# flo-audio/flo

Hardware: AMD Instinct MI355X
Metric: Msamples/s encoded (44.1k stereo, q=high) (higher is better)
Workload: dtype f32

## Files before the change

### flo_amd/csrc/context.cpp

```cpp
#include <cstdio>
#include <cstdlib>
#include <cstring>

#include "ctx_internal.hpp"

thread_local std::string g_create_err;

int fail(flo_ctx *c, int code, const std::string &msg) {
    if (c) c->err = msg;
    return code;
}

extern "C" const char *flo_last_create_error(void) { return g_create_err.c_str(); }
extern "C" const char *flo_last_error(const flo_ctx *ctx) { return ctx ? ctx->err.c_str() : "null context"; }
extern "C" void flo_free(void *p) { free(p); }

extern "C" int flo_ctx_create(int device, flo_ctx **out) {
    if (!out) return FLO_ERR_ARG;
    *out = nullptr;
    int n = 0;
    hipError_t e = hipGetDeviceCount(&n);
    if (e != hipSuccess || n == 0) {
        g_create_err = std::string("no HIP device available: ") + (e != hipSuccess ? hipGetErrorString(e) : "count = 0") +
                       " (libflo_hip has no CPU fallback)";
        return FLO_ERR_DEVICE;
    }
    if (device < 0 || device >= n) {
        g_create_err = "device index out of range";
        return FLO_ERR_ARG;
    }
    flo_ctx *c = new flo_ctx();
    c->device = device;
    int prev_dev = -1;
    hipGetDevice(&prev_dev);
    auto restore = [&] {
        if (prev_dev >= 0 && prev_dev != device) hipSetDevice(prev_dev);
    };
    if ((e = hipSetDevice(device)) != hipSuccess || (e = hipGetDeviceProperties(&c->prop, device)) != hipSuccess ||
        (e = hipStreamCreateWithFlags(&c->stream, hipStreamNonBlocking)) != hipSuccess) {
        g_create_err = std::string("device init failed: ") + hipGetErrorString(e);
        delete c;
        restore();
        return FLO_ERR_DEVICE;
    }
    if (std::string(c->prop.gcnArchName).find("gfx950") == std::string::npos) {
        g_create_err = std::string("device is ") + c->prop.gcnArchName + ", this library carries gfx950 code only";
        hipStreamDestroy(c->stream);
        delete c;
        restore();
        return FLO_ERR_DEVICE;
    }
    {
        std::string serr;
        c->stager = stager_create(serr);
    }
    if (const char *e2 = getenv("FLO_RESERVE_CUS")) {
        const int v = atoi(e2);
// ... 97 lines not shown
        if (t->host.sample_rate == sr && t->host.quality == q) {
            *out = t;
            return FLO_OK;
        }
    TableSet *t = new TableSet();
    build_lossy_tables(sr, q, t->host);
    const LossyTablesHost &h = t->host;
    struct Part {
        const void *src;
        size_t bytes;
        size_t off;
    };
    std::vector<Part> parts;
    size_t total = 0;
    auto add = [&](const void *p, size_t b) {
        total = (total + 255) & ~(size_t)255;
        parts.push_back({p, b, total});
        total += b;
        return parts.size() - 1;
    };
    size_t i_ext = add(h.pack_ext.data(), h.pack_ext.size() * 4);
    size_t i_pack = add(h.pack.data(), h.pack.size() * 4), i_athdb = add(h.ath_db.data(), h.ath_db.size() * 4),
           i_band = add(h.band.data(), h.band.size()), i_bc = add(h.band_count.data(), h.band_count.size() * 4),
           i_s10 = add(h.s10d.data(), h.s10d.size() * 4), i_lb = add(h.lane_bnd.data(), h.lane_bnd.size() * 4),
           i_ls = add(h.lane_slot0.data(), h.lane_slot0.size() * 4), i_bs = add(h.band_slot0.data(), h.band_slot0.size() * 4),
           i_win = add(h.window.data(), h.window.size() * 4);
    hipError_t e = hipMalloc(&t->blob, total);
    if (e != hipSuccess) {
        delete t;
        return fail(c, FLO_ERR_NOMEM, std::string("hipMalloc tables: ") + hipGetErrorString(e));
    }
    std::vector<uint8_t> stage(total, 0);
    for (auto &p : parts) memcpy(stage.data() + p.off, p.src, p.bytes);
    e = hipMemcpy(t->blob, stage.data(), total, hipMemcpyHostToDevice);
    if (e != hipSuccess) {
        hipFree(t->blob);
        delete t;
        return fail(c, FLO_ERR_DEVICE, std::string("hipMemcpy tables: ") + hipGetErrorString(e));
    }
    auto P = [&](size_t i) { return (const char *)t->blob + parts[i].off; };
    t->dev.pack = (const float4 *)P(i_pack);
    t->dev.pack_g = t->dev.pack;
    t->dev.pack_ext = (const float4 *)P(i_ext);
    t->dev.ath_db = (const float *)P(i_athdb);
    t->dev.band = (const uint8_t *)P(i_band);
    t->dev.band_count = (const float *)P(i_bc);
    t->dev.s10d = (const float *)P(i_s10);
    t->dev.lane_bnd = (const uint32_t *)P(i_lb);
    t->dev.lane_slot0 = (const uint32_t *)P(i_ls);
    t->dev.band_slot0 = (const uint32_t *)P(i_bs);
    t->dev_window = (const float *)P(i_win);
    t->dev.max_band_slots = h.max_band_slots;
    t->dev.dirty = h.dirty;
    t->dev.smr_thr = h.smr_threshold;
    t->dev.q_transparent = h.q_transparent;
    if (h.n_slots > kSlotCap || h.max_band_slots > 64) {
        hipFree(t->blob);
        delete t;
        return fail(c, FLO_ERR_ARG, "band segment table exceeds capacity");
    }
    c->tables.push_back(t);
    *out = t;
    return FLO_OK;
}

int ctx_stager(flo_ctx *c) {
    if (c->stager && c->up_stream) return FLO_OK;
    if (c->stager) {
        HIPCHK(c, hipStreamCreateWithFlags(&c->up_stream, hipStreamNonBlocking));
        HIPCHK(c, hipStreamCreateWithFlags(&c->down_stream, hipStreamNonBlocking));
        return FLO_OK;
    }
    std::string err;
    c->stager = stager_create(err);
    if (!c->stager) return fail(c, FLO_ERR_NOMEM, err);
    HIPCHK(c, hipStreamCreateWithFlags(&c->up_stream, hipStreamNonBlocking));
    HIPCHK(c, hipStreamCreateWithFlags(&c->down_stream, hipStreamNonBlocking));
    return FLO_OK;
}

extern "C" int flo_ctx_reserve_cus(flo_ctx *c, int n) {
    if (!c || n < 0 || n >= c->prop.multiProcessorCount) return FLO_ERR_ARG;
    c->reserve_cus = n;
    return FLO_OK;
}
extern "C" int flo_ctx_upload_path(flo_ctx *c, char *name, size_t cap, double *direct_gbs, double *ring_gbs) {
    if (!c) return FLO_ERR_ARG;
    int rc = ctx_stager(c);
    if (rc != FLO_OK) return rc;
    const char *n = stager_upload_choice(c->stager, direct_gbs, ring_gbs);
    if (name && cap) snprintf(name, cap, "%s", n);
    return FLO_OK;
}
extern "C" int flo_ctx_reserved_cus(flo_ctx *c) { return c ? (c->reserve_cus > 0 ? c->reserve_cus : 0) : -1; }
```

### flo_amd/csrc/encode_plan.hpp

```cpp
#pragma once
#include <cstddef>
#include <cstdint>

namespace flo {

constexpr size_t kFewClips = 64;
constexpr size_t kFusedCompactClips = 16;
constexpr size_t kCoefHandoverBytes = (size_t)256 << 20;
constexpr uint32_t kDirty44k = 0xBDBEu;

enum class LossyForm : uint8_t {
    Chain2q = 5,
    Chain = 1,
    Frames = 2,
};
enum class Chain2qKernel : uint8_t {
    None,
    InCoeffs,
    Debug,
    Dirty44k,
    Generic,
};
enum class ChainKernel : uint8_t {
    None,
    Mono,
    MonoExact,
    Stereo,
    StereoExact,
};
enum class FrameKernel : uint8_t {
    None,
    Mono1, Mono2, Mono2Exact,
    Stereo1, Stereo2, Stereo2Exact,
    Pair1, Pair2,
    Pair2FromCoef,
    Multi1, Multi2, Multi2Exact,
};
enum class CompactKernel : uint8_t {
    None,
    Fused,
    Offsets1024,
    Offsets256,
};

struct LossyPlanInput {
    int which = 0;
    int force_path = 0;
    unsigned ch = 0;
    size_t n_clips = 0;
    uint64_t total_frames = 0;
    bool exact = false, in_coeffs = false;
    bool debug = false;
    uint32_t dirty = 0;
    bool tail_crc = true;
    int chain2q_clips = 0;
};

struct LossyPlan {
    LossyForm form = LossyForm::Chain;
    Chain2qKernel chain2q = Chain2qKernel::None;
    int chain2q_clips = 0;
    ChainKernel chain = ChainKernel::None;
// ... 21 lines not shown
```

### flo_amd/csrc/lossy_device.hpp

```cpp
#pragma once
#include <hip/hip_runtime.h>
#include <stdint.h>

#include "pack_rows.h"

namespace flo {


struct LossyDevTables {
    const float4 *pack;
    const float4 *pack_g;
    const float4 *pack_ext;
    const float *ath_db;
    const uint8_t *band;
    const float *band_count;
    const float *s10d;
    const uint32_t *lane_bnd;
    const uint32_t *lane_slot0;
    const uint32_t *band_slot0;
    int max_band_slots;
    uint32_t dirty;
    float smr_thr;
    int q_transparent;
};

constexpr int kXchStride = 9;
constexpr int kXchFloats = 64 * kXchStride * 2;
#ifdef FLO_COEF_PAD16
constexpr int kCoefFloats = 1280;
#else
constexpr int kCoefFloats = 1152;
#endif
constexpr int kSlotCap = 96;
constexpr int kFrameCap = 4352;

template <int CH>
struct WaveLds {
    union {
        float xch[CH][kXchFloats];
        float coef[CH][kCoefFloats];
        int16_t qbuf[CH][1024];
    } u;
    float2 slots[CH][kSlotCap + 64 + 1];
    float2 bandv[CH][32];
    float band_s[CH][32];
};

__device__ __forceinline__ float4 pack_row(const float4 *p) {
    typedef float v4f __attribute__((ext_vector_type(4)));
    v4f v = *reinterpret_cast<const v4f *>(p);
    asm("" : "+v"(v));
    return make_float4(v.x, v.y, v.z, v.w);
}

__device__ __forceinline__ int lane_id() { return (int)(threadIdx.x & 63); }
__device__ __forceinline__ int lane_id_opaque() {
    int l = (int)(threadIdx.x & 63);
    asm volatile("" : "+v"(l));
    return l;
}

__device__ __forceinline__ void wave_sync() {
    asm volatile("" ::: "memory");
    __builtin_amdgcn_wave_barrier();
    asm volatile("" ::: "memory");
}
__device__ __forceinline__ void lds_barrier() {
    asm volatile("s_waitcnt lgkmcnt(0)\n\ts_barrier" ::: "memory");
}

__device__ __forceinline__ float max_raw(float a, float b) {
    float r;
    asm("v_max_f32 %0, %1, %2" : "=v"(r) : "v"(a), "v"(b));
    return r;
}
__device__ __forceinline__ float max_abs_raw(float a, float b) {
// ... 954 lines not shown
#pragma unroll
    for (int g = 0; g < 4; g++) {
        const float4 al4 = T.pack[(kRowAth + g) * 64 + lane];
        const float4 bo4 = R.bo4[g];
        const float al[4] = {al4.x, al4.y, al4.z, al4.w};
        const uint32_t bo[4] = {__float_as_uint(bo4.x), __float_as_uint(bo4.y), __float_as_uint(bo4.z), __float_as_uint(bo4.w)};
        v4f tb[4];
#pragma unroll
        for (int k = 0; k < 4; k++) tb[k] = *reinterpret_cast<const lds_f4 *>((uintptr_t)(ts0 + 2u * bo[k]));
        int v[2][4];
        float t[2][4];
#pragma unroll
        for (int k = 0; k < 4; k++) {
            const v2f x = c[4 * g + k];
            const v2f xsc = x * (v2f){tb[k].z, tb[k].w};
            uint32_t h0, h1;
            asm("v_bfi_b32 %0, %1, %2, %3" : "=v"(h0) : "s"(sgn_mask), "v"(phalf), "v"(x.x));
            asm("v_bfi_b32 %0, %1, %2, %3" : "=v"(h1) : "s"(sgn_mask), "v"(phalf), "v"(x.y));
            const v2f rs = xsc + (v2f){__uint_as_float(h0), __uint_as_float(h1)};
            v[0][k] = cvt_rz(rs.x);
            v[1][k] = cvt_rz(rs.y);
            t[0][k] = max_raw(tb[k].x, al[k]);
            t[1][k] = max_raw(tb[k].y, al[k]);
        }
#pragma unroll
        for (int ch = 0; ch < 2; ch++)
#pragma unroll
            for (int k2 = 0; k2 < 2; k2++) {
                const float xe = ch ? c[4 * g + 2 * k2].y : c[4 * g + 2 * k2].x;
                const float xo = ch ? c[4 * g + 2 * k2 + 1].y : c[4 * g + 2 * k2 + 1].x;
                uint32_t r;
                asm("v_cmp_gt_f32_e64 vcc, |%1|, %2\n\t"
                    "v_cndmask_b32_e32 %0, 0, %3, vcc\n\t"
                    "v_cmp_gt_f32_e64 vcc, |%4|, %5\n\t"
                    "v_cndmask_b32_sdwa %0, 0, %6, vcc dst_sel:WORD_1 dst_unused:UNUSED_PRESERVE src0_sel:DWORD src1_sel:DWORD"
                    : "=&v"(r)
                    : "v"(xe), "v"(t[ch][2 * k2]), "v"(v[ch][2 * k2]), "v"(xo), "v"(t[ch][2 * k2 + 1]), "v"(v[ch][2 * k2 + 1])
                    : "vcc");
                xs[ch][2 * g + k2] = r;
            }
    }
}

typedef float v4f __attribute__((ext_vector_type(4)));
template <int TSOFF>
__device__ __forceinline__ void quantise_nat(const v4f (&cf)[8], const uint32_t (&ts_a)[16], const float (&athn)[16],
                                             const uint32_t alive, const uint32_t (&blk)[8], uint32_t (&xd)[2][8]) {
    typedef __attribute__((address_space(3))) v4f lds_f4;
    const uint32_t sgn_mask = 0x7FFFFFFFu;
    uint32_t phalf = 0x3EFFFFFFu;
    asm volatile("" : "+v"(phalf));
    auto block = [&](const int k, const v4f t0, const v4f t1, uint32_t &out0, uint32_t &out1) __attribute__((always_inline)) {
        const v2f x0 = {cf[k].x, cf[k].y}, x1 = {cf[k].z, cf[k].w};
        const v2f s0 = x0 * (v2f){t0.z, t0.w}, s1 = x1 * (v2f){t1.z, t1.w};
        uint32_t h00, h01, h10, h11;
        asm("v_bfi_b32 %0, %1, %2, %3" : "=v"(h00) : "s"(sgn_mask), "v"(phalf), "v"(x0.x));
        asm("v_bfi_b32 %0, %1, %2, %3" : "=v"(h01) : "s"(sgn_mask), "v"(phalf), "v"(x0.y));
        asm("v_bfi_b32 %0, %1, %2, %3" : "=v"(h10) : "s"(sgn_mask), "v"(phalf), "v"(x1.x));
        asm("v_bfi_b32 %0, %1, %2, %3" : "=v"(h11) : "s"(sgn_mask), "v"(phalf), "v"(x1.y));
        const v2f r0 = s0 + (v2f){__uint_as_float(h00), __uint_as_float(h01)};
        const v2f r1 = s1 + (v2f){__uint_as_float(h10), __uint_as_float(h11)};
        const int v0[2] = {cvt_rz(r0.x), cvt_rz(r0.y)}, v1[2] = {cvt_rz(r1.x), cvt_rz(r1.y)};
        const float a0 = athn[2 * k], a1 = athn[2 * k + 1];
        const float th0[2] = {max_raw(t0.x, a0), max_raw(t0.y, a0)}, th1[2] = {max_raw(t1.x, a1), max_raw(t1.y, a1)};
        uint32_t r[2];
#pragma unroll
        for (int ch = 0; ch < 2; ch++) {
            const float xe = ch ? x0.y : x0.x, xo = ch ? x1.y : x1.x;
            asm("v_cmp_gt_f32_e64 vcc, |%1|, %2\n\t"
                "v_cndmask_b32_e32 %0, 0, %3, vcc\n\t"
                "v_cmp_gt_f32_e64 vcc, |%4|, %5\n\t"
                "v_cndmask_b32_sdwa %0, 0, %6, vcc dst_sel:WORD_1 dst_unused:UNUSED_PRESERVE src0_sel:DWORD src1_sel:DWORD"
                : "=&v"(r[ch])
                : "v"(xe), "v"(th0[ch]), "v"(v0[ch]), "v"(xo), "v"(th1[ch]), "v"(v1[ch])
                : "vcc");
        }
        out0 = r[0];
        out1 = r[1];
    };
#pragma unroll
    for (int g = 0; g < 4; g++) {
        uint32_t o00 = 0u, o01 = 0u, o10 = 0u, o11 = 0u;
        if (alive & (blk[2 * g] | blk[2 * g + 1])) {
            v4f tb[4];
#pragma unroll
            for (int j = 0; j < 4; j++) tb[j] = *reinterpret_cast<const lds_f4 *>((uintptr_t)(ts_a[4 * g + j] + (uint32_t)TSOFF));
            if (alive & blk[2 * g]) block(2 * g, tb[0], tb[1], o00, o01);
            if (alive & blk[2 * g + 1]) block(2 * g + 1, tb[2], tb[3], o10, o11);
        }
        xd[0][2 * g] = o00, xd[1][2 * g] = o01;
        xd[0][2 * g + 1] = o10, xd[1][2 * g + 1] = o11;
    }
}

__device__ __forceinline__ uint32_t nonzero_mask16(const int (&q)[16]) {
    uint32_t m = 0;
#pragma unroll
    for (int e = 0; e < 16; e++) m |= (q[e] != 0 ? 1u : 0u) << e;
    return m;
}
__device__ __forceinline__ uint32_t nonzero_mask16_packed(const uint32_t (&x)[8], const uint32_t (&hi)[8]) {
    uint32_t m = 0;
#pragma unroll
    for (int k = 0; k < 8; k++) {
        m |= ((x[k] & 0xFFFFu) != 0u ? 1u : 0u) << (2 * k);
        m |= (hi[k] != 0u ? 1u : 0u) << (2 * k + 1);
    }
    return m;
}
__device__ __forceinline__ uint32_t wave_incl_sum(uint32_t x) {
    int v = (int)x;
    v += dpp_i<0x111>(0, v);
    v += dpp_i<0x112>(0, v);
    v += dpp_i<0x114>(0, v);
    v += dpp_i<0x118>(0, v);
    v += dpp_i<0x142, 0xA>(0, v);
    v += dpp_i<0x143, 0xC>(0, v);
    return (uint32_t)v;
}

struct SparsePlan {
    uint32_t M;
    int nn;
    int nz_end;
    uint32_t cross_cnt;
    uint32_t off0;
    uint32_t total;
};

__device__ __forceinline__ void sparse_plan_m(const int lane, const uint32_t m, SparsePlan &P) {
    const uint32_t prev_m = (uint32_t)dpp_i<0x138>(0, (int)m);
    const uint32_t prev_nz = (prev_m >> 15) & 1u;
    uint32_t zs = ~m & ((m << 1) | prev_nz) & 0xFFFFu;
    if (lane == 0 && !(m & 1u)) zs |= 1u;
    const int base = 16 * lane;
    const uint32_t inv = ~m & 0xFFFFu;
    const int first_nz = m ? base + __builtin_ctz(m) : 1024;
    const int first_z = inv ? base + __builtin_ctz(inv) : 1024;
    const int last_z = inv ? base + 31 - __builtin_clz(inv) : -1;
    const unsigned long long has_nz = __ballot(m != 0u), has_z = __ballot(inv != 0u);
    const unsigned long long nz_above = (has_nz >> 1) >> lane, z_above = (has_z >> 1) >> lane;
// ... 405 lines not shown
```

### flo_amd/csrc/lossy_kernels.hip

```cpp
#include <assert.h>
#include <stdlib.h>

#include <mutex>
#include <set>
#include <type_traits>
#include <utility>

#include "crc_device.hpp"
#include "lossy_device.hpp"
#include "lossy_kernels.hpp"
#include "../../include/flo_synth.h"

#ifndef FLO_ABLATE
#define FLO_ABLATE 0
#endif
#ifndef FLO_SKIP
#define FLO_SKIP 0
#endif
#ifndef FLO_ABLATE3
#define FLO_ABLATE3 0
#endif
#define FLO_KEEP(x) asm volatile("" ::"v"(x))
#ifdef FLO_STAMPS
#define STAMP(i)                                                                                  \
// ... 283 lines not shown
        STAMP(4);
#if FLO_ABLATE >= 2
        FLO_KEEP(P[0].total); FLO_KEEP(P[0].off0); FLO_KEEP(P[0].M); FLO_KEEP(sfw[0]);
        for (int e = 0; e < 16; e++) FLO_KEEP(q[0][e]);
        return;
#endif
        uint32_t tot[2];
        if (NW > 1) {
            if (ln == 0) cs.tot[w] = P[0].total;
            pair_sync(cs.cnt, w, ++step);
            STAMP(5);
            tot[0] = cs.tot[0];
            tot[1] = cs.tot[1];
        } else {
            wave_sync();
            tot[0] = P[0].total;
            tot[1] = 0u;
        }
        if (ptid < (int)pend) stage[ptid] = (uint8_t)tailb;
        const uint32_t flen = emit_frame<1>(ln, stage + pend, NW, w, tot, sfw, P, q);
        STAMP(6);
#if FLO_ABLATE >= 1
        FLO_KEEP(flen);
        return;
#endif
        if (NW > 1) pair_sync(cs.cnt, w, ++step); else wave_sync();
        STAMP(7);
        if (ptid == 0) A.frame_size[frame0 + h] = flen;
        const uint32_t have = pend + flen;
        const uint32_t n16 = have >> 4;
        const uint4 *src = reinterpret_cast<const uint4 *>(stage);
        uint4 *dst = reinterpret_cast<uint4 *>(gout + written);
        for (uint32_t i = ptid; i < n16; i += 64 * NW) dst[i] = src[i];
        pend = have & 15u;
        tailb = (ptid < (int)pend) ? stage[(n16 << 4) + ptid] : 0u;
        written += (unsigned long long)n16 << 4;
        STAMP(8);
    };
    for (unsigned h = 0; h < hops; h += 2) {
        frame_body(h, ae, ao, be, bo);
        if (h + 1 < hops) frame_body(h + 1, be, bo, ae, ao);
    }
    if (ptid < (int)pend) gout[written + ptid] = (uint8_t)tailb;
    if (ptid == 0) A.clip_bytes[clip] = written + pend;
#ifdef FLO_STAMPS
    if (A.dbg_stamps && lane == 0)
        for (int i = 0; i < 14; i++) A.dbg_stamps[((unsigned long long)clip * NW + w) * 16 + i] = st_sum[i];
#endif
}

template <int SLEEP = 1>
__device__ __forceinline__ void wait_counter(const uint32_t *p, uint32_t want) {
    const uint32_t a = (uint32_t)(uintptr_t)p;
    uint32_t seen;
    do {
        asm volatile("ds_read_b32 %0, %1\n\ts_waitcnt lgkmcnt(0)" : "=v"(seen) : "v"(a) : "memory");
        if (seen >= want) break;
        __builtin_amdgcn_s_sleep(SLEEP);
    } while (true);
}
__device__ __forceinline__ uint32_t peek_counter(const uint32_t *p) {
    typedef volatile __attribute__((address_space(3))) uint32_t lds_vu32;
    return *reinterpret_cast<lds_vu32 *>((uintptr_t)(uint32_t)(uintptr_t)p);
}
__device__ __forceinline__ void set_counter(uint32_t *p, uint32_t v) {
    const uint32_t a = (uint32_t)(uintptr_t)p;
    asm volatile("ds_write_b32 %0, %1" ::"v"(a), "v"(v) : "memory");
}

#ifndef FLO_C2X_THREADS
#define FLO_C2X_THREADS 768
#endif
#ifdef FLO_MARKS
#define FLO_MARK(x) asm volatile("; MARK " x ::: "memory")
#else
#define FLO_MARK(x)
#endif

struct Clip2qLds {
    union {
        float4 xch4[kXch4];
        float2 coef2[kCoef2];
    } u;
    float4 slot[kSlots];
    float4 ts[2][32];
    __attribute__((aligned(16))) uint8_t stage[kFrameCap + 64 + 256];
    uint16_t sfwh[2][2][32];
    uint32_t alive[2][2];
    uint32_t pad2[4];
    uint32_t packtab[kPackTabDwords];
    uint32_t coef_ready;
    uint32_t ts_ready;
    uint32_t consumed;
    uint32_t clip_seq;
    uint32_t clip_cur;
    uint32_t pad[3];
};
static_assert(sizeof(Clip2qLds) % 16 == 0, "clip LDS block keeps 16-byte alignment");
constexpr int kPackBytesHotT = kPackRowsHotT * 64 * 16;

#ifndef FLO_PSLEEP
#define FLO_PSLEEP 1
#endif
static_assert(sizeof(Clip2qLds::u) >= 8 * 256 * sizeof(uint32_t), "the tail's CRC tables fit the exchange buffer");

__device__ __forceinline__ void tail_publish(const LossyArgs &A, const unsigned clip, const int lane) {
    asm volatile("s_waitcnt vmcnt(0)" ::: "memory");
    if (lane == 0) {
        __builtin_amdgcn_fence(__ATOMIC_RELEASE, "agent");
        asm volatile("s_waitcnt vmcnt(0)" ::: "memory");
        const unsigned slot = __hip_atomic_fetch_add(A.next_clip + 1, 1u, __ATOMIC_RELAXED, __HIP_MEMORY_SCOPE_AGENT);
        if (slot < (unsigned)A.n_clips)
// ... 37 lines not shown
                if (h < (unsigned)A.n_clips) e = __hip_atomic_load(A.done_q + h, __ATOMIC_RELAXED, __HIP_MEMORY_SCOPE_AGENT);
            }
        }
        const unsigned tag = (unsigned)__builtin_amdgcn_readfirstlane((int)(unsigned)(e >> 32));
        clip = (unsigned)__builtin_amdgcn_readfirstlane((int)(unsigned)e);
        if (tag != A.epoch || clip >= (unsigned)A.n_clips) return;
        __builtin_amdgcn_fence(__ATOMIC_ACQUIRE, "agent");
        asm volatile("s_waitcnt vmcnt(0)" ::: "memory");
        total = __hip_atomic_load(A.clip_bytes + clip, __ATOMIC_RELAXED, __HIP_MEMORY_SCOPE_AGENT);
    }
}

template <bool COEFFS, uint32_t DIRTY, bool DBG>
__global__ __launch_bounds__(FLO_C2X_THREADS) void lossy_chain2q_kernel(LossyArgs A, int clips_per_wg) {
    extern __shared__ __attribute__((aligned(16))) uint8_t lds_raw[];
    const int tid = (int)threadIdx.x;
    const int lane = tid & 63;
    {
        float4 *dstp = reinterpret_cast<float4 *>(lds_raw);
        for (int i = tid; i < kPackRowsHotT * 64; i += (int)blockDim.x) dstp[i] = A.T.pack[i];
        for (int i = tid; i < clips_per_wg; i += (int)blockDim.x) {
            Clip2qLds &c0 = *reinterpret_cast<Clip2qLds *>(lds_raw + kPackBytesHotT + (size_t)i * sizeof(Clip2qLds));
            c0.coef_ready = 0;
            c0.ts_ready = 0;
            c0.consumed = 0;
            c0.clip_seq = 0;
        }
        if (A.clear_next && blockIdx.x == 0 && tid == 0)
            A.clear_next[0] = A.clear_next[1] = A.clear_next[2] = 0;
    }
    __syncthreads();
    const int wv = __builtin_amdgcn_readfirstlane(tid >> 6);
    const int cl = wv % clips_per_wg;
    Clip2qLds &cs = *reinterpret_cast<Clip2qLds *>(lds_raw + kPackBytesHotT + (size_t)cl * sizeof(Clip2qLds));
    uint32_t fbase = 0, seq = 0;
    if (wv >= clips_per_wg) {
#ifndef FLO_PRIO_P
#define FLO_PRIO_P 1
#endif
        __builtin_amdgcn_s_setprio(FLO_PRIO_P);
        typedef __attribute__((address_space(3))) v4f lds_v4f;
        float athn[16];
        uint32_t ts_a[16];
        {
            const uint32_t ts0 = (uint32_t)(uintptr_t)cs.ts[0];
#pragma unroll
            for (int q = 0; q < 4; q++) {
                const float4 a4 = A.T.pack[(kRowAthN + q) * 64 + lane];
                const float4 b4 = A.T.pack[(kRowBoN + q) * 64 + lane];
                athn[4 * q + 0] = a4.x, athn[4 * q + 1] = a4.y, athn[4 * q + 2] = a4.z, athn[4 * q + 3] = a4.w;
                ts_a[4 * q + 0] = ts0 + __float_as_uint(b4.x), ts_a[4 * q + 1] = ts0 + __float_as_uint(b4.y);
                ts_a[4 * q + 2] = ts0 + __float_as_uint(b4.z), ts_a[4 * q + 3] = ts0 + __float_as_uint(b4.w);
            }
        }
        const uint32_t *const blk_g = reinterpret_cast<const uint32_t *>(A.T.pack + kRowBlk * 64);
        const uint32_t cf_a = (uint32_t)(uintptr_t)cs.u.coef2 + 16u * (uint32_t)lane + 16u * ((uint32_t)lane >> 3);
        uint8_t *const stage = cs.stage;
        const uint32_t tab_a = (uint32_t)(uintptr_t)cs.packtab;
        v4f cf[8];
        bool have = false;
        unsigned done_clip = ~0u;
        unsigned long long done_bytes = 0;
        for (;;) {
            unsigned got = 0;
            if (lane == 0) got = atomicAdd(A.next_clip, 1u);
            const unsigned clip = (unsigned)__builtin_amdgcn_readfirstlane((int)got);
            if (lane == 0) cs.clip_cur = clip;
            set_counter(&cs.clip_seq, ++seq);
            if (A.crc_ready) {
                if (clip >= (unsigned)A.n_clips) {
                    tail_crc(A, reinterpret_cast<uint32_t *>(&cs.u), lane, done_clip, done_bytes);
                    return;
                }
                if (done_clip != ~0u) tail_publish(A, done_clip, lane);
            }
            if (clip >= (unsigned)A.n_clips) return;
            const unsigned hops = A.clip_hops[clip];
            const unsigned long long frame0 = A.clip_frame0[clip];
            uint8_t *gout = A.out + A.out_off[clip];
            unsigned long long written = 0;
            uint32_t pend = 0, tailb = 0;
#ifdef FLO_STAMPS
            unsigned long long st_sum[16] = {0, 0, 0, 0, 0, 0, 0, 0, 0, 0, 0, 0, 0, 0, 0, 0}, st_last;
            asm volatile("s_memtime %0\n\ts_waitcnt lgkmcnt(0)" : "=s"(st_last)::"memory");
#endif
            for (unsigned h = 0; h < hops; h++) {
                const int ln = lane_id_opaque();
                const uint32_t g = fbase + h;
                auto take_next = [&]() __attribute__((always_inline)) {
                    if (!have && (uint32_t)__builtin_amdgcn_readfirstlane((int)peek_counter(&cs.coef_ready)) >= g + 2) {
#pragma unroll
                        for (int k = 0; k < 8; k++) cf[k] = *reinterpret_cast<const lds_v4f *>((uintptr_t)(cf_a + 1152u * (uint32_t)k));
                        set_counter(&cs.consumed, g + 2);
                        have = true;
                    }
                };
                uint32_t blk[8];
                {
                    const uint32_t *bp = blk_g;
                    asm volatile("" : "+s"(bp));
#pragma unroll
                    for (int q = 0; q < 8; q++) blk[q] = bp[q];
                }
                if (!have) {
                    wait_counter<FLO_PSLEEP>(&cs.coef_ready, g + 1);
#pragma unroll
                    for (int k = 0; k < 8; k++) cf[k] = *reinterpret_cast<const lds_v4f *>((uintptr_t)(cf_a + 1152u * (uint32_t)k));
                    set_counter(&cs.consumed, g + 1);
                }
                STAMP(0);
#ifdef FLO_STAMPS
                const unsigned long long st_frame0 = st_last;
#endif
                wait_counter<FLO_PSLEEP>(&cs.ts_ready, g + 1);
                STAMP(5);
                const uint32_t par = g & 1u;
                const uint32_t sfw_both = cs.sfwh[par][ln >> 5][ln & 31];
                const uint32_t alive = (uint32_t)__builtin_amdgcn_readfirstlane((int)(cs.alive[par][0] | cs.alive[par][1]));
                uint32_t xd[2][8];
#if (FLO_SKIP & 64) == 0
                if (par) quantise_nat<512>(cf, ts_a, athn, alive, blk, xd);
                else quantise_nat<0>(cf, ts_a, athn, alive, blk, xd);
#else
#pragma unroll
                for (int q = 0; q < 8; q++) { xd[0][q] = __float_as_uint(cf[q].x) & alive & 0x00010001u; xd[1][q] = __float_as_uint(cf[q].y) & blk[q] & 0x00010001u; }
#endif
                have = false;
                take_next();
                STAMP(1);
                if (DBG && A.dbg_q) {
#pragma unroll
                    for (int ch = 0; ch < 2; ch++) {
                        uint32_t *dq = reinterpret_cast<uint32_t *>(A.dbg_q + ((frame0 + h) * 2 + ch) * 1024);
#pragma unroll
                        for (int k = 0; k < 8; k++) dq[64 * k + ln] = xd[ch][k];
                    }
                }
                if (ln < (int)pend) stage[ln] = (uint8_t)tailb;
                uint8_t *f = stage + pend;
                const uint32_t f_a = (uint32_t)(uintptr_t)f;
                if ((ln & 31) < 25) {
                    uint8_t *p = f + 12 + 50 * (ln >> 5) + 2 * (ln & 31);
                    lds_st8<0>(p, sfw_both);
                    lds_st8<1>(p, sfw_both >> 8);
                }
                uint32_t tot[2];
                uint32_t pos = 112;
#pragma unroll
                for (int ch = 0; ch < 2; ch++) {
#if (FLO_SKIP & 32) == 0
                    uint32_t t = sparse_item_pack(ln, xd[ch], f_a + pos + 4u, tab_a);
#ifdef FLO_STAMPS
                    if (t == kSparseFallback) st_sum[6] += 1;
#endif
                    if (t == kSparseFallback) t = sparse_block_pack(ln, xd[ch], f_a + pos + 4u, tab_a);
// ... 1020 lines not shown
    hipError_t e = hipGetDevice(&dev);
    if (e != hipSuccess) return (int)e;
    std::lock_guard<std::mutex> g(mu);
    if (done.count({dev, fn})) return 0;
    e = hipFuncSetAttribute(fn, hipFuncAttributeMaxDynamicSharedMemorySize, 160 * 1024);
    if (e != hipSuccess) return (int)e;
    done.insert({dev, fn});
    return 0;
}

int chain_clips_per_wg(int n_clips) {
    int g = (n_clips + 255) / 256;
    const int gmax = (int)((160 * 1024 - kPackBytes) / sizeof(ClipLds));
    if (g > gmax) g = gmax;
    if (g * 2 * 64 > 768) g = 6;
    return g < 1 ? 1 : g;
}

template <int NW, bool EXACT>
static int launch_chain_t(const LossyArgs &A, hipStream_t s) {
    const int g = chain_clips_per_wg(A.n_clips);
    const size_t lds = kPackBytes + (size_t)g * sizeof(ClipLds);
    if (int rc = allow_big_lds(reinterpret_cast<const void *>(&lossy_chain_kernel<NW, EXACT>))) return rc;
    const unsigned wgs = (unsigned)((A.n_clips + g - 1) / g);
    hipLaunchKernelGGL((lossy_chain_kernel<NW, EXACT>), dim3(wgs), dim3(64 * NW * g), lds, s, A, g);
    FLO_LAUNCH_CHECK();
    return 0;
}

int chain2q_clips_per_wg(int n_clips) {
    int g = (n_clips + 255) / 256;
    const int gmax = (int)((160 * 1024 - kPackBytesHotT) / sizeof(Clip2qLds));
    if (g > gmax) g = gmax;
    if (g > FLO_C2X_THREADS / 128) g = FLO_C2X_THREADS / 128;
    return g < 1 ? 1 : g;
}
template <bool COEFFS, uint32_t DIRTY, bool DBG>
static int launch_chain2q_t(const LossyArgs &A, int clips, hipStream_t s) {
    int g = chain2q_clips_per_wg(A.n_clips);
    if (clips >= 1 && clips <= FLO_C2X_THREADS / 128) g = clips;
    const size_t lds = kPackBytesHotT + (size_t)g * sizeof(Clip2qLds);
    if (int rc = allow_big_lds(reinterpret_cast<const void *>(&lossy_chain2q_kernel<COEFFS, DIRTY, DBG>))) return rc;
    unsigned wgs = (unsigned)((A.n_clips + g - 1) / g);
    if (A.n_cus > 0 && wgs > (unsigned)A.n_cus) wgs = (unsigned)A.n_cus;
    hipLaunchKernelGGL((lossy_chain2q_kernel<COEFFS, DIRTY, DBG>), dim3(wgs), dim3(128 * g), lds, s, A, g);
    FLO_LAUNCH_CHECK();
    return 0;
}
int launch_lossy_chain2q(const LossyArgs &A, const LossyPlan &P, hipStream_t s) {
    assert(P.form == LossyForm::Chain2q && A.nch == 2 && !A.exact);
    switch (P.chain2q) {
    case Chain2qKernel::InCoeffs: return launch_chain2q_t<true, 0xFFFFu, true>(A, P.chain2q_clips, s);
    case Chain2qKernel::Debug: return launch_chain2q_t<false, 0xFFFFu, true>(A, P.chain2q_clips, s);
    case Chain2qKernel::Dirty44k: return launch_chain2q_t<false, kDirty44k, false>(A, P.chain2q_clips, s);
    case Chain2qKernel::Generic: return launch_chain2q_t<false, 0xFFFFu, false>(A, P.chain2q_clips, s);
    default: return -1;
    }
}
int launch_lossy_chain(const LossyArgs &A, const LossyPlan &P, hipStream_t s) {
    switch (P.chain) {
    case ChainKernel::Mono: return launch_chain_t<1, false>(A, s);
    case ChainKernel::MonoExact: return launch_chain_t<1, true>(A, s);
    case ChainKernel::Stereo: return launch_chain_t<2, false>(A, s);
    case ChainKernel::StereoExact: return launch_chain_t<2, true>(A, s);
    default: return -1;
    }
}
int launch_lossy_frames_pass(const LossyArgs &A, FrameKernel k, hipStream_t s) {
    dim3 g((unsigned)A.total_frames), b(64);
    const size_t dynb = (size_t)A.slot_bytes + 256 + (size_t)A.nch * 2048;
    switch (k) {
    case FrameKernel::Mono1: hipLaunchKernelGGL((lossy_frame_kernel<1, 1, false>), g, b, 0, s, A); break;
    case FrameKernel::Mono2: hipLaunchKernelGGL((lossy_frame_kernel<1, 2, false>), g, b, 0, s, A); break;
    case FrameKernel::Mono2Exact: hipLaunchKernelGGL((lossy_frame_kernel<1, 2, true>), g, b, 0, s, A); break;
    case FrameKernel::Stereo1: hipLaunchKernelGGL((lossy_frame_kernel<2, 1, false>), g, b, 0, s, A); break;
    case FrameKernel::Stereo2: hipLaunchKernelGGL((lossy_frame_kernel<2, 2, false>), g, b, 0, s, A); break;
    case FrameKernel::Stereo2Exact: hipLaunchKernelGGL((lossy_frame_kernel<2, 2, true>), g, b, 0, s, A); break;
    case FrameKernel::Pair1: hipLaunchKernelGGL((lossy_frame2x_kernel<1>), g, b, 0, s, A); break;
    case FrameKernel::Pair2: hipLaunchKernelGGL((lossy_frame2x_kernel<2>), g, b, 0, s, A); break;
    case FrameKernel::Pair2FromCoef: hipLaunchKernelGGL((lossy_frame2x_kernel<2, true>), g, b, 0, s, A); break;
    case FrameKernel::Multi1: hipLaunchKernelGGL((lossy_frame_n_kernel<1, false>), g, b, dynb, s, A); break;
    case FrameKernel::Multi2: hipLaunchKernelGGL((lossy_frame_n_kernel<2, false>), g, b, dynb, s, A); break;
    case FrameKernel::Multi2Exact: hipLaunchKernelGGL((lossy_frame_n_kernel<2, true>), g, b, dynb, s, A); break;
    default: return -1;
    }
    FLO_LAUNCH_CHECK();
    return 0;
}
int launch_lossy_stream_pass(const LossyArgs &A, int pass, hipStream_t s) {
    dim3 g((unsigned)A.total_frames), b(64);
    const size_t dynb = (size_t)A.slot_bytes + 256 + (size_t)A.nch * 2048;
    constexpr int S1 = 1 | kStreamStep, S2 = 2 | kStreamStep;
    if (A.nch == 1) {
        if (pass == 1) hipLaunchKernelGGL((lossy_frame_kernel<1, S1, false>), g, b, 0, s, A);
        else if (A.exact) hipLaunchKernelGGL((lossy_frame_kernel<1, S2, true>), g, b, 0, s, A);
        else hipLaunchKernelGGL((lossy_frame_kernel<1, S2, false>), g, b, 0, s, A);
    } else if (A.nch == 2 && A.exact) {
        if (pass == 1) hipLaunchKernelGGL((lossy_frame_kernel<2, S1, false>), g, b, 0, s, A);
        else hipLaunchKernelGGL((lossy_frame_kernel<2, S2, true>), g, b, 0, s, A);
    } else if (A.nch == 2) {
        if (pass == 1) hipLaunchKernelGGL((lossy_frame2x_kernel<S1>), g, b, 0, s, A);
        else hipLaunchKernelGGL((lossy_frame2x_kernel<S2>), g, b, 0, s, A);
    } else if (A.nch <= kMaxLossyChannels) {
        if (pass == 1) hipLaunchKernelGGL((lossy_frame_n_kernel<S1, false>), g, b, dynb, s, A);
        else if (A.exact) hipLaunchKernelGGL((lossy_frame_n_kernel<S2, true>), g, b, dynb, s, A);
        else hipLaunchKernelGGL((lossy_frame_n_kernel<S2, false>), g, b, dynb, s, A);
    } else {
// ... 74 lines not shown
```

Before: 658,000.

## Specialise 44k block masks as constants and tighten quantiser and wait-loop codegen

For the 44.1k dirty-band kernel variant, the per-frame block masks become compile-time constants instead of being loaded from global memory. The host checks the table against these constants and falls back to the generic kernel on a mismatch. The quantiser block is rewritten as one interleaved asm sequence that uses separate SGPR masks, to cut vcc serialisation. The counter wait loop moves into scalar-branch asm using readfirstlane, which avoids divergent exec-mask handling. A diagnostic script for counting issue slots is also added.

```diff
diff --git a/diag/issue_slots.py b/diag/issue_slots.py
--- /dev/null
+++ b/diag/issue_slots.py
@@ -0,0 +1,118 @@
+#!/usr/bin/env python3
+import collections
+import re
+import sys
+
+BLOCK = re.compile(r"^(\.LBB\d+_\d+):|^; %bb\.\d+:")
+
+
+def classify(op):
+    if op == "s_nop":
+        return "s_nop"
+    if op.startswith("v_"):
+        return "vector"
+    if op.startswith("ds_"):
+        return "lds"
+    if op.startswith("s_waitcnt"):
+        return "wait"
+    if op.startswith(("global_", "buffer_", "flat_", "scratch_")):
+        return "vmem"
+    if op.startswith(("s_load", "s_buffer_load")):
+        return "smem"
+    if op.startswith("s_"):
+        return "scalar"
+    return None
+
+
+def blocks_of(lines):
+    out = [(None, "", [])]
+    for l in lines:
+        m = BLOCK.match(l)
+        if m:
+            out.append((m.group(1), l.split(";", 1)[1] if ";" in l else "", []))
+            continue
+        s = l.strip()
+        if not s:
+            continue
+        if s.startswith(";"):
+            if not s.startswith(";;#") and not out[-1][2]:
+                out[-1] = (out[-1][0], out[-1][1] + " " + s, out[-1][2])
+            continue
+        if s.startswith((".", "//")) or s.endswith(":"):
+            continue
+        out[-1][2].append(s)
+    return out
+
+
+def loop_blocks(blocks, header):
+    pat = re.compile(r"\b" + re.escape(header.lstrip(".L")) + r"\b")
+    return [b for b in blocks if b[0] == header or pat.search(b[1])]
+
+
+def depth2_header(block):
+    if "This Loop Header: Depth=2" in block[1]:
+        return block[0]
+    m = re.search(r"Header=(BB\d+_\d+) Depth=2", block[1]) or re.search(r"Parent Loop (BB\d+_\d+) Depth=2", block[1])
+    return ".L" + m.group(1) if m else None
+
+
+def histogram(insts):
+    c, br, ops = collections.Counter(), collections.Counter(), collections.Counter()
+    for s in insts:
+        op = s.split()[0]
+        k = classify(op)
+        if k is None:
+            continue
+        c[k] += 1
+        ops[op] += 1
+        if op.startswith("s_cbranch") or op == "s_branch":
+            br[op] += 1
+        elif op.startswith(("s_and_saveexec", "s_or_saveexec", "s_andn2_saveexec")):
+            br[op] += 1
+        elif op in ("s_or_b64", "s_andn2_b64", "s_and_b64", "s_mov_b64") and re.match(r"\S+\s+exec\b", s):
+            br[op + " exec"] += 1
+    return c, br, ops
+
+
+def report(name, insts, div, watch):
+    c, br, ops = histogram(insts)
+    row = "  ".join(f"{k} {c[k] / div:g}" for k in ("vector", "scalar", "s_nop", "lds", "vmem", "smem", "wait"))
+    print(f"{name}: {row}  | issued (without waits) {sum(v for k, v in c.items() if k != 'wait') / div:g}")
+    print("    branch forms: " + (", ".join(f"{k} {v / div:g}" for k, v in sorted(br.items())) or "none"))
+    print("    " + ", ".join(f"{k} {ops[k] / div:g}" for k in watch))
+
+
+def main():
+    path = sys.argv[1]
+    want = sys.argv[2] if len(sys.argv) > 2 else "lossy_chain2q_kernelILb0ELj48574ELb0EE"
+    lines = open(path).read().split("\n")
+    start = next(i for i, l in enumerate(lines) if l.startswith("_Z") and want in l and ":" in l.split(";")[0])
+    end = next(i for i in range(start, len(lines)) if ".size" in lines[i] and want in lines[i])
+    blocks = blocks_of(lines[start:end])
+    whole = [s for b in blocks for s in b[2]]
+    c, _, ops = histogram(whole)
+    print(f"{want}: {sum(c.values())} instructions, s_nop {c['s_nop']}, s_and_saveexec_b64 {ops['s_and_saveexec_b64']}, "
+          f"v_mov_b32 {ops['v_mov_b32_e32']}, flat_load_dwordx4 {ops['flat_load_dwordx4']}")
+    first = next(i for i, b in enumerate(blocks) if any(s.startswith("v_cmp_ne_u16") for s in b[2]))
+    ph = depth2_header(blocks[first])
+    insts = []
+    for b in loop_blocks(blocks, ph):
+        stop = next((j for j, s in enumerate(b[2]) if s.startswith("v_cmp_ne_u16")), None)
+        insts += b[2] if stop is None else b[2][:stop]
+        if stop is not None:
+            break
+    report("packer frame loop up to the first sparse-pack compare", insts, 1,
+           ("v_mov_b32_e32", "v_add_u32_e32", "v_cmp_ne_u32_e32", "v_cmp_ne_u32_e64", "v_and_b32_e32", "v_bitop3_b32", "flat_load_dwordx4",
+            "s_and_b32", "v_readfirstlane_b32"))
+    per_loop = collections.Counter()
+    for b in blocks:
+        h = depth2_header(b)
+        if h:
+            per_loop[h] += sum(s.startswith("v_pk_fma_f32") for s in b[2])
+    th = per_loop.most_common(1)[0][0]
+    insts = [s for b in loop_blocks(blocks, th) for s in b[2]]
+    report("transform frame body (half the loop unrolled by two)", insts, 2, ("v_pk_fma_f32", "v_pk_mul_f32", "v_pk_add_f32", "v_mov_b32_e32"))
+
+
+if __name__ == "__main__":
+    main()
diff --git a/flo_amd/csrc/context.cpp b/flo_amd/csrc/context.cpp
--- a/flo_amd/csrc/context.cpp
+++ b/flo_amd/csrc/context.cpp
@@ -3,6 +3,7 @@
 #include <cstring>
 
 #include "ctx_internal.hpp"
+#include "encode_plan.hpp"
 
 thread_local std::string g_create_err;
 
@@ -206,6 +207,7 @@
     t->dev_window = (const float *)P(i_win);
     t->dev.max_band_slots = h.max_band_slots;
     t->dev.dirty = h.dirty;
+    t->dev.blk44k = memcmp(&h.pack[(size_t)kRowBlk * 64 * 4], flo::kBlk44k, sizeof(flo::kBlk44k)) == 0;
     t->dev.smr_thr = h.smr_threshold;
     t->dev.q_transparent = h.q_transparent;
     if (h.n_slots > kSlotCap || h.max_band_slots > 64) {
diff --git a/flo_amd/csrc/encode_plan.hpp b/flo_amd/csrc/encode_plan.hpp
--- a/flo_amd/csrc/encode_plan.hpp
+++ b/flo_amd/csrc/encode_plan.hpp
@@ -8,6 +8,7 @@
 constexpr size_t kFusedCompactClips = 16;
 constexpr size_t kCoefHandoverBytes = (size_t)256 << 20;
 constexpr uint32_t kDirty44k = 0xBDBEu;
+constexpr uint32_t kBlk44k[8] = {0x0000FFFFu, 0x000F8000u, 0x00380000u, 0x00600000u, 0x00C00000u, 0x01800000u, 0x01000000u, 0x01000000u};
 
 enum class LossyForm : uint8_t {
     Chain2q = 5,
diff --git a/flo_amd/csrc/lossy_device.hpp b/flo_amd/csrc/lossy_device.hpp
--- a/flo_amd/csrc/lossy_device.hpp
+++ b/flo_amd/csrc/lossy_device.hpp
@@ -22,6 +22,7 @@
     uint32_t dirty;
     float smr_thr;
     int q_transparent;
+    int blk44k;
 };
 
 constexpr int kXchStride = 9;
@@ -1082,41 +1083,53 @@
     asm volatile("" : "+v"(phalf));
     auto block = [&](const int k, const v4f t0, const v4f t1, uint32_t &out0, uint32_t &out1) __attribute__((always_inline)) {
         const v2f x0 = {cf[k].x, cf[k].y}, x1 = {cf[k].z, cf[k].w};
+        auto half_signed = [&](const float x) __attribute__((always_inline)) {
+            return __uint_as_float((phalf & sgn_mask) | (__float_as_uint(x) & ~sgn_mask));
+        };
         const v2f s0 = x0 * (v2f){t0.z, t0.w}, s1 = x1 * (v2f){t1.z, t1.w};
-        uint32_t h00, h01, h10, h11;
-        asm("v_bfi_b32 %0, %1, %2, %3" : "=v"(h00) : "s"(sgn_mask), "v"(phalf), "v"(x0.x));
-        asm("v_bfi_b32 %0, %1, %2, %3" : "=v"(h01) : "s"(sgn_mask), "v"(phalf), "v"(x0.y));
-        asm("v_bfi_b32 %0, %1, %2, %3" : "=v"(h10) : "s"(sgn_mask), "v"(phalf), "v"(x1.x));
-        asm("v_bfi_b32 %0, %1, %2, %3" : "=v"(h11) : "s"(sgn_mask), "v"(phalf), "v"(x1.y));
-        const v2f r0 = s0 + (v2f){__uint_as_float(h00), __uint_as_float(h01)};
-        const v2f r1 = s1 + (v2f){__uint_as_float(h10), __uint_as_float(h11)};
-        const int v0[2] = {cvt_rz(r0.x), cvt_rz(r0.y)}, v1[2] = {cvt_rz(r1.x), cvt_rz(r1.y)};
-        const float a0 = athn[2 * k], a1 = athn[2 * k + 1];
-        const float th0[2] = {max_raw(t0.x, a0), max_raw(t0.y, a0)}, th1[2] = {max_raw(t1.x, a1), max_raw(t1.y, a1)};
-        uint32_t r[2];
-#pragma unroll
-        for (int ch = 0; ch < 2; ch++) {
-            const float xe = ch ? x0.y : x0.x, xo = ch ? x1.y : x1.x;
-            asm("v_cmp_gt_f32_e64 vcc, |%1|, %2\n\t"
-                "v_cndmask_b32_e32 %0, 0, %3, vcc\n\t"
-                "v_cmp_gt_f32_e64 vcc, |%4|, %5\n\t"
-                "v_cndmask_b32_sdwa %0, 0, %6, vcc dst_sel:WORD_1 dst_unused:UNUSED_PRESERVE src0_sel:DWORD src1_sel:DWORD"
-                : "=&v"(r[ch])
-                : "v"(xe), "v"(th0[ch]), "v"(v0[ch]), "v"(xo), "v"(th1[ch]), "v"(v1[ch])
-                : "vcc");
-        }
-        out0 = r[0];
-        out1 = r[1];
+        const v2f r0 = s0 + (v2f){half_signed(x0.x), half_signed(x0.y)};
+        const v2f r1 = s1 + (v2f){half_signed(x1.x), half_signed(x1.y)};
+        uint32_t o0, o1;
+        float w0, w1, w2, w3;
+        unsigned long long m0, m1;
+        asm("v_max_f32 %[w0], %[t00], %[a0]\n\t"
+            "v_max_f32 %[w1], %[t01], %[a0]\n\t"
+            "v_max_f32 %[w2], %[t10], %[a1]\n\t"
+            "v_cvt_i32_f32 %[o0], %[r00]\n\t"
+            "v_cmp_gt_f32_e64 %[m0], |%[x00]|, %[w0]\n\t"
+            "v_cmp_gt_f32_e64 %[m1], |%[x01]|, %[w1]\n\t"
+            "v_cmp_gt_f32_e64 vcc, |%[x10]|, %[w2]\n\t"
+            "v_cvt_i32_f32 %[w0], %[r10]\n\t"
+            "v_cndmask_b32_e64 %[o0], 0, %[o0], %[m0]\n\t"
+            "v_max_f32 %[w3], %[t11], %[a1]\n\t"
+            "v_cndmask_b32_sdwa %[o0], 0, %[w0], vcc dst_sel:WORD_1 dst_unused:UNUSED_PRESERVE src0_sel:DWORD src1_sel:DWORD\n\t"
+            "v_cmp_gt_f32_e64 vcc, |%[x11]|, %[w3]\n\t"
+            "v_cvt_i32_f32 %[o1], %[r01]\n\t"
+            "v_cvt_i32_f32 %[w1], %[r11]\n\t"
+            "v_cndmask_b32_e64 %[o1], 0, %[o1], %[m1]\n\t"
+            "v_cndmask_b32_sdwa %[o1], 0, %[w1], vcc dst_sel:WORD_1 dst_unused:UNUSED_PRESERVE src0_sel:DWORD src1_sel:DWORD"
+            : [o0] "=&v"(o0), [o1] "=&v"(o1), [m0] "=&s"(m0), [m1] "=&s"(m1), [w0] "=&v"(w0), [w1] "=&v"(w1), [w2] "=&v"(w2), [w3] "=&v"(w3)
+            : [t00] "v"(t0.x), [t01] "v"(t0.y), [t10] "v"(t1.x), [t11] "v"(t1.y), [r00] "v"(r0.x), [r01] "v"(r0.y), [r10] "v"(r1.x),
+              [r11] "v"(r1.y), [a0] "v"(athn[2 * k]), [a1] "v"(athn[2 * k + 1]), [x00] "v"(x0.x), [x01] "v"(x0.y), [x10] "v"(x1.x),
+              [x11] "v"(x1.y)
+            : "vcc");
+        out0 = o0;
+        out1 = o1;
     };
 #pragma unroll
     for (int g = 0; g < 4; g++) {
-        uint32_t o00 = 0u, o01 = 0u, o10 = 0u, o11 = 0u;
-        if (alive & (blk[2 * g] | blk[2 * g + 1])) {
+        uint32_t o00, o01, o10, o11;
+        const bool live0 = (alive & blk[2 * g]) != 0u, live1 = (alive & blk[2 * g + 1]) != 0u;
+        if (live0 || live1) {
             v4f tb[4];
 #pragma unroll
-            for (int j = 0; j < 4; j++) tb[j] = *reinterpret_cast<const lds_f4 *>((uintptr_t)(ts_a[4 * g + j] + (uint32_t)TSOFF));
-            if (alive & blk[2 * g]) block(2 * g, tb[0], tb[1], o00, o01);
-            if (alive & blk[2 * g + 1]) block(2 * g + 1, tb[2], tb[3], o10, o11);
+            for (int j = 0; j < 4; j++) tb[j] = *reinterpret_cast<const lds_f4 *>((uintptr_t)ts_a[4 * g + j] + (uintptr_t)TSOFF);
+            if (live0) block(2 * g, tb[0], tb[1], o00, o01);
+            else o00 = o01 = 0u;
+            if (live1) block(2 * g + 1, tb[2], tb[3], o10, o11);
+            else o10 = o11 = 0u;
+        } else {
+            o00 = o01 = o10 = o11 = 0u;
         }
         xd[0][2 * g] = o00, xd[1][2 * g] = o01;
         xd[0][2 * g + 1] = o10, xd[1][2 * g + 1] = o11;
diff --git a/flo_amd/csrc/lossy_kernels.hip b/flo_amd/csrc/lossy_kernels.hip
--- a/flo_amd/csrc/lossy_kernels.hip
+++ b/flo_amd/csrc/lossy_kernels.hip
@@ -359,12 +359,19 @@
 template <int SLEEP = 1>
 __device__ __forceinline__ void wait_counter(const uint32_t *p, uint32_t want) {
     const uint32_t a = (uint32_t)(uintptr_t)p;
-    uint32_t seen;
-    do {
-        asm volatile("ds_read_b32 %0, %1\n\ts_waitcnt lgkmcnt(0)" : "=v"(seen) : "v"(a) : "memory");
-        if (seen >= want) break;
-        __builtin_amdgcn_s_sleep(SLEEP);
-    } while (true);
+    uint32_t seen, seen_s;
+    asm volatile(".Lwait_counter_%=:\n\t"
+                 "ds_read_b32 %0, %2\n\t"
+                 "s_waitcnt lgkmcnt(0)\n\t"
+                 "v_readfirstlane_b32 %1, %0\n\t"
+                 "s_cmp_ge_u32 %1, %3\n\t"
+                 "s_cbranch_scc1 .Lwait_counter_done_%=\n\t"
+                 "s_sleep %4\n\t"
+                 "s_branch .Lwait_counter_%=\n"
+                 ".Lwait_counter_done_%=:"
+                 : "=&v"(seen), "=&s"(seen_s)
+                 : "v"(a), "s"(want), "n"(SLEEP)
+                 : "memory", "scc");
 }
 __device__ __forceinline__ uint32_t peek_counter(const uint32_t *p) {
     typedef volatile __attribute__((address_space(3))) uint32_t lds_vu32;
@@ -508,6 +515,8 @@
                 ts_a[4 * q + 0] = ts0 + __float_as_uint(b4.x), ts_a[4 * q + 1] = ts0 + __float_as_uint(b4.y);
                 ts_a[4 * q + 2] = ts0 + __float_as_uint(b4.z), ts_a[4 * q + 3] = ts0 + __float_as_uint(b4.w);
             }
+#pragma unroll
+            for (int e = 0; e < 16; e++) asm volatile("" : "+v"(ts_a[e]));
         }
         const uint32_t *const blk_g = reinterpret_cast<const uint32_t *>(A.T.pack + kRowBlk * 64);
         const uint32_t cf_a = (uint32_t)(uintptr_t)cs.u.coef2 + 16u * (uint32_t)lane + 16u * ((uint32_t)lane >> 3);
@@ -552,11 +561,15 @@
                     }
                 };
                 uint32_t blk[8];
-                {
-                    const uint32_t *bp = blk_g;
+                if constexpr (DIRTY == kDirty44k) {
+#pragma unroll
+                    for (int q = 0; q < 8; q++) blk[q] = kBlk44k[q];
+                } else {
+                    typedef const __attribute__((address_space(4))) uint32_t *const_u32_p;
+                    uintptr_t bp = (uintptr_t)blk_g;
                     asm volatile("" : "+s"(bp));
 #pragma unroll
-                    for (int q = 0; q < 8; q++) blk[q] = bp[q];
+                    for (int q = 0; q < 8; q++) blk[q] = reinterpret_cast<const_u32_p>(bp)[q];
                 }
                 if (!have) {
                     wait_counter<FLO_PSLEEP>(&cs.coef_ready, g + 1);
@@ -1683,7 +1696,9 @@
     switch (P.chain2q) {
     case Chain2qKernel::InCoeffs: return launch_chain2q_t<true, 0xFFFFu, true>(A, P.chain2q_clips, s);
     case Chain2qKernel::Debug: return launch_chain2q_t<false, 0xFFFFu, true>(A, P.chain2q_clips, s);
-    case Chain2qKernel::Dirty44k: return launch_chain2q_t<false, kDirty44k, false>(A, P.chain2q_clips, s);
+    case Chain2qKernel::Dirty44k:
+        if (A.T.blk44k) return launch_chain2q_t<false, kDirty44k, false>(A, P.chain2q_clips, s);
+        [[fallthrough]];
     case Chain2qKernel::Generic: return launch_chain2q_t<false, 0xFFFFu, false>(A, P.chain2q_clips, s);
     default: return -1;
     }
```

After: 665,800 (median of 6 runs). 1.01x the previous value.
